# musyoku/chainer-speech-recognition

Measured on AMD Instinct MI355X. Metric: utterances/sec (T=1000, 40x3 feat, |V|~3000) CTC train step, higher is better.
Workload: dtype bf16

## Files before the change

### chainer-speech-recognition_amd/asr/_lib.py

```python
import ctypes
import os

import torch

_HERE = os.path.dirname(os.path.abspath(__file__))
_ACT = os.environ.get("ASR_ACT", "").lower()
LIB_PATH = os.environ.get("ASR_HIP_LIB") or os.path.join(os.path.dirname(_HERE),
                                                        "libasr_hip_f16.so" if _ACT in ("f16", "fp16", "float16", "half") else "libasr_hip.so")

_lib = None


def act_dtype():
    return torch.float16 if lib().asr_act_dtype() else torch.bfloat16


def debug_flag(key, default):
    for item in os.environ.get("ASR_DEBUG", "").split(","):
        k, _, v = item.strip().partition("=")
        if k == key and v:
            return int(v)
    return default

c_void_p, c_int, c_float, c_size_t = ctypes.c_void_p, ctypes.c_int, ctypes.c_float, ctypes.c_size_t
c_longlong = ctypes.c_longlong

SIGNATURES = {
    "asr_version": (c_int, []),
    "asr_act_dtype": (c_int, []),
    "asr_stream_delay": (c_int, [c_void_p, c_int]),
    "asr_occupy_cus": (c_int, [c_void_p, c_int, c_int, c_int]),
    "asr_stream_traffic": (c_int, [c_void_p, c_int, c_int, c_int, c_void_p, c_longlong]),
    "asr_ctc_workspace_bytes": (c_size_t, [c_int] * 5),
    "asr_ctc_forward": (c_int, [c_void_p] * 6 + [c_int] * 5 + [c_void_p] * 3 + [c_size_t]),
    "asr_ctc_forward_lse": (c_int, [c_void_p] * 6 + [c_int] * 5 + [c_void_p] * 3 + [c_size_t, c_void_p]),
    "asr_ctc_backward": (c_int, [c_void_p] * 3 + [c_int] * 5 + [c_void_p, c_int, c_float, c_void_p, c_void_p, c_size_t]),
    "asr_ctc_loss_grad": (c_int, [c_void_p] * 6 + [c_int] * 5 + [c_float] + [c_void_p] * 4 + [c_size_t]),
    "asr_ctc_nbest_workspace_bytes": (c_size_t, [c_int] * 5),
    "asr_ctc_nbest_forward": (c_int, [c_void_p] * 5 + [c_int] * 6 + [c_void_p, c_void_p, c_size_t]),
    "asr_ctc_nbest_backward": (c_int, [c_void_p] * 3 + [c_int] * 5 + [c_void_p] * 3 + [c_size_t]),
    "asr_specgram": (c_int, [c_void_p, c_void_p, c_int, c_void_p, c_longlong] + [c_int] * 4 + [c_float, c_void_p, c_void_p, c_int,
                               c_void_p, c_void_p, c_int, c_void_p]),
    "asr_mel_bands_bytes": (c_size_t, []),
    "asr_mel_bands": (c_int, [c_void_p, c_void_p, c_int, c_int, c_void_p, c_size_t]),
    "asr_specgram_bands": (c_int, [c_void_p, c_void_p, c_int, c_void_p, c_longlong] + [c_int] * 4 + [c_float, c_void_p, c_void_p, c_int,
                                     c_void_p, c_void_p, c_int, c_void_p, c_void_p]),
    "asr_logmel": (c_int, [c_void_p] * 3 + [c_longlong, c_int, c_int, c_void_p]),
    "asr_deltas": (c_int, [c_void_p] * 3 + [c_int] * 4 + [c_void_p] * 3),
    "asr_batchnorm_stats": (c_int, [c_void_p, c_void_p, c_longlong, c_int, c_float, c_float] + [c_void_p] * 5),
    "asr_rsqrt_eps": (c_int, [c_void_p, c_void_p, c_float, c_void_p, c_int]),
    "asr_batchnorm_fwd": (c_int, [c_void_p] * 6 + [c_longlong, c_int, c_void_p]),
    "asr_batchnorm_bwd": (c_int, [c_void_p] * 6 + [c_longlong, c_int] + [c_void_p] * 4),
    "asr_cmn_pspec": (c_int, [c_void_p] * 3 + [c_int] * 3),
    "asr_add_white_noise": (c_int, [c_void_p] * 3 + [c_longlong, c_int, c_void_p, ctypes.c_ulonglong]),
    "asr_augment_specgram": (c_int, [c_void_p] * 5 + [c_int] * 4 + [c_void_p]),
    "asr_running_stats_update": (c_int, [c_void_p] * 3 + [c_int] * 3 + [c_longlong] + [c_void_p] * 4),
    "asr_normalize_bcmt": (c_int, [c_void_p] * 4 + [c_int] * 3),
    "asr_argmax_rows": (c_int, [c_void_p, c_void_p, c_int, c_int, c_int, c_void_p]),
    "asr_ctc_collapse": (c_int, [c_void_p] * 3 + [c_int] * 4 + [c_void_p] * 2),
    "asr_edit_distance": (c_int, [c_void_p, c_void_p, c_void_p, c_int, c_void_p, c_void_p, c_int, c_int, c_void_p]),
    "asr_ctc_beam_workspace_bytes": (c_size_t, [c_int] * 5),
    "asr_ctc_beam_search": (c_int, [c_void_p] * 3 + [c_int] * 6 + [c_float, c_void_p, c_size_t] + [c_void_p] * 3),
    "asr_ngram_score": (c_int, [c_void_p] * 2 + [c_int, c_void_p, c_void_p] + [c_int] * 3 + [c_void_p] * 2 + [c_int] * 4 + [c_void_p] * 2),
    "asr_ctc_beam_lm_workspace_bytes": (c_size_t, [c_int] * 5),
    "asr_ctc_beam_search_lm": (c_int, [c_void_p] * 3 + [c_int] * 6 + [c_float, c_void_p, c_int, c_void_p, c_void_p] + [c_int] * 5
                               + [c_float, c_float, c_void_p, c_size_t] + [c_void_p] * 5),
    "asr_gram_ctc_beam_workspace_bytes": (c_size_t, [c_int] * 5),
    "asr_gram_ctc_beam_search": (c_int, [c_void_p] * 3 + [c_int] * 6 + [c_float, c_void_p, c_void_p, c_size_t] + [c_void_p] * 3),
# ... 145 lines not shown
```

### chainer-speech-recognition_amd/asr/_ops.py

```python
import os

import torch

from . import _lib
from ._lib import check, ptr, stream

BF16 = _lib.act_dtype()
F32 = torch.float32


def _is_bf16(t):
    if t.dtype == BF16:
        return 1
    if t.dtype == F32:
        return 0
    raise TypeError("expected float32 or bfloat16, got %s" % t.dtype)


def gemm_nt(a, b, bias=None, out_dtype=BF16, out=None):
    assert a.dtype == BF16 and b.dtype == BF16 and a.dim() == 2 and b.dim() == 2
    assert a.stride(1) == 1 and b.stride(1) == 1 and a.shape[1] == b.shape[1]
    M, K = a.shape
    N = b.shape[0]
    if out is None:
# ... 271 lines not shown
    y = torch.empty((rows, D), dtype=out_dtype, device=x.device)
    mean = torch.empty(rows, dtype=F32, device=x.device)
    rstd = torch.empty(rows, dtype=F32, device=x.device)
    if want_lse:
        assert x.dtype == F32 and out_dtype == F32 and _lib.lib().asr_layernorm_fwd_lse_ok(D, C)
        lse = torch.empty(rows, dtype=F32, device=x.device)
        rc = _lib.lib().asr_layernorm_fwd_lse(stream(), ptr(x), ptr(y), ptr(gamma), ptr(beta), ptr(mean), ptr(rstd), ptr(lse), rows, D)
        check(rc, "asr_layernorm_fwd_lse")
        return y, mean, rstd, lse
    rc = _lib.lib().asr_layernorm_fwd(stream(), ptr(x), _is_bf16(x), ptr(y), _is_bf16(y), ptr(gamma), ptr(beta),
                                      ptr(mean), ptr(rstd), rows, D, C)
    check(rc, "asr_layernorm_fwd")
    return y, mean, rstd


def layernorm_bwd(x, dy, gamma, mean, rstd, C, dx_dtype, dgamma=None, dbeta=None, need_dx=True):
    rows, D = x.shape
    dy = dy.contiguous()
    dx = torch.empty((rows, D), dtype=dx_dtype, device=x.device) if need_dx else None
    lib = _lib.lib()
    if x.dtype == F32 and dy.dtype == F32 and C % 4 == 0:
        nbytes = lib.asr_layernorm_bwd_rows_ws_bytes(rows, D)
        if nbytes > 0:
            ws = torch.empty(nbytes, dtype=torch.uint8, device=x.device) if dgamma is not None else None
            rc = lib.asr_layernorm_bwd_rows(stream(), ptr(x), ptr(dy), ptr(gamma), ptr(mean), ptr(rstd), ptr(dx),
                                            _is_bf16(dx) if need_dx else 0, ptr(dgamma), ptr(dbeta), rows, D, C, ptr(ws), nbytes)
            check(rc, "asr_layernorm_bwd_rows")
            return dx
    rc = lib.asr_layernorm_bwd(stream(), ptr(x), _is_bf16(x), ptr(dy), _is_bf16(dy), ptr(gamma), ptr(mean),
                               ptr(rstd), ptr(dx), _is_bf16(dx) if need_dx else 0, ptr(dgamma), ptr(dbeta),
                               rows, D, C)
    check(rc, "asr_layernorm_bwd")
    return dx


CALLS = {}


def layernorm_ctc_bwd(x, gamma, beta, mean, rstd, T, B, dx_dtype, dgamma, dbeta, need_dx, recipes, dxsum=None):
    rows, V = x.shape
    assert x.dtype == F32 and x.is_contiguous() and rows == T * B and 1 <= len(recipes) <= 2
    CALLS["layernorm_ctc_bwd"] = CALLS.get("layernorm_ctc_bwd", 0) + 1
    lib = _lib.lib()
    dx = torch.empty((rows, V), dtype=dx_dtype, device=x.device) if need_dx else None
    nbytes = lib.asr_layernorm_ctc_bwd_ws_bytes(T, B, V)
    ws = torch.empty(nbytes, dtype=torch.uint8, device=x.device) if dgamma is not None else None
    args = []
    for r in (recipes + recipes)[:2]:
        args += [ptr(r["ws"]), int(r["Lmax"]), int(r["gram"]), ptr(r["x_len"]), ptr(r["gy"]), int(r["gy_per_utt"]), float(r["scale"])]
    rc = lib.asr_layernorm_ctc_bwd(stream(), ptr(x), ptr(gamma), ptr(beta), ptr(mean), ptr(rstd), ptr(dx), _is_bf16(dx) if need_dx else 0,
                                   ptr(dgamma), ptr(dbeta), T, B, V, ptr(ws), nbytes, len(recipes), *args, ptr(dxsum))
    check(rc, "asr_layernorm_ctc_bwd")
    return dx


GRU_MODE = [int(os.environ.get("ASR_GRU_MODE", "0"))]


_SYNC = {}
_STATUS = {}


def _sync_buffer(dev, nbytes):
    key = (dev.index, torch.cuda.current_stream(dev).cuda_stream)
    buf = _SYNC.get(key)
    if buf is None or buf.numel() * 4 < nbytes:
# ... 687 lines not shown
```

### chainer-speech-recognition_amd/asr/functions.py

```python
import math
import os

import torch

from . import _ops
from ._lib import debug_flag as _lib_debug
from .link import grad_buffer, grads_queued

BF16, F32 = _ops.BF16, torch.float32


_SIDE = {"streams": {}, "origins": {}, "enabled": True, "dirty": set(), "keep": [], "keep_bytes": 0,
         "join_before_recurrence": _lib_debug("side_join", 0) != 0}
_KEEP_LIMIT = 512
_KEEP_BYTES_LIMIT = int(_lib_debug("side_keep_gb", 48)) << 30


def side_stream():
    if not _SIDE["enabled"]:
        return None
    cur = torch.cuda.current_stream()
    key = cur.cuda_stream
    st = _SIDE["streams"].get(key)
    if st is None:
        st = _SIDE["streams"][key] = torch.cuda.Stream(priority=_lib_debug("side_priority", 0))
        _SIDE["origins"][key] = cur
    return st


def side_streams():
    return list(_SIDE["streams"].values())


def join_side_stream():
    cur = torch.cuda.current_stream()
    for key, st in _SIDE["streams"].items():
        cur.wait_stream(st)
        origin = _SIDE["origins"].get(key)
        if origin is not None and origin.cuda_stream != cur.cuda_stream:
            origin.wait_stream(st)
    _SIDE["dirty"].clear()
    release_side_keeps()


def release_side_keeps(to_allocator=False):
    keep = _SIDE["keep"]
    if to_allocator:
        for t, st in keep:
            t.record_stream(st)
    del keep[:]
    _SIDE["keep_bytes"] = 0


def _empty_chip_for_recurrence():
    if not _SIDE["join_before_recurrence"] or not _SIDE["dirty"]:
        return
    cur = torch.cuda.current_stream()
    for st in _SIDE["dirty"]:
        cur.wait_stream(st)
    _SIDE["dirty"].clear()


class _OnSide(object):

# ... 53 lines not shown
    z = _ZERO.get(device)
    if z is None:
        z = _ZERO[device] = torch.zeros(1, dtype=F32, device=device)
    return z.reshape((1,) * len(shape)).expand(shape)


def _is_zero_token(t):
    z = _ZERO.get(t.device)
    return z is not None and t.data_ptr() == z.data_ptr()


def _producer_box(x2, attr="_asr_mailbox", hops=12, dtype=F32):
    if x2.dtype != dtype or not x2.is_contiguous():
        return None
    node = x2.grad_fn
    for _ in range(hops):
        if node is None:
            return None
        box = getattr(node, attr, None)
        if box is not None:
            return box if (box.ptr == x2.data_ptr() and box.numel == x2.numel()) else None
        if not type(node).__name__.startswith(_VIEW_NODES) or len(node.next_functions) != 1:
            return None
        node = node.next_functions[0][0]
    return None


def _producer_mailbox(x2):
    return _producer_box(x2, "_asr_mailbox", 8)


FUSE_CTC_INTO_LAYERNORM = [True]
LAST_FUSED_RECIPES = [0]


class _CtcBox(object):
    __slots__ = ("ptr", "numel", "shape", "recipes", "lse")

    def __init__(self, y, T, B, V, lse=None):
        self.ptr, self.numel, self.shape, self.recipes, self.lse = y.data_ptr(), y.numel(), (T, B, V), [], lse

    def post(self, recipe):
        self.recipes.append(recipe)
        return len(self.recipes) == 1

    def take(self):
        r, self.recipes = self.recipes, []
        return r


def ctc_box_of(xs):
    if not FUSE_CTC_INTO_LAYERNORM[0] or xs.dim() != 3:
        return None
    box = _producer_box(xs, "_asr_ctc_box")
    return box if (box is not None and box.shape == tuple(xs.shape)) else None


def _incoming_bf16(ctx, gy, width):
    box = getattr(ctx, "_asr_mailbox", None)
    extra = box.take() if box is not None else None
    if extra is not None and _is_zero_token(gy):
        return extra.reshape(-1, width), None
    gy = gy.contiguous()
    if gy.dtype != BF16:
        gy = _ops.cast_bf16(gy.reshape(-1, width))
    gy = gy.reshape(-1, width)
    if extra is not None:
        return _ops.add_bf16(gy, extra.reshape(-1, width)), gy
    return gy, gy


def _take_bias_done(ctx):
    done = False
# ... 690 lines not shown
    y = _SppMax.apply(p, int(pyramid_height))
    parts, o = [], 0
    for l in range(int(pyramid_height)):
        n = 4 ** l
        parts.append(y[:, o:o + n, :].permute(0, 2, 1).reshape(B, C * n))
        o += n
    return torch.cat(parts, dim=1).reshape(B, -1, 1, 1)


class _GaussianNoise(torch.autograd.Function):
    @staticmethod
    def forward(ctx, p, std, seed):
        return _ops.gaussian_noise(p, std, seed)

    @staticmethod
    def backward(ctx, gy):
        return gy, None, None


def gaussian_noise(x, std):
    if not train_mode[0]:
        return x
    p, back = _phys_any(x)
    _dropout_counter[0] += 1
    seed = (torch.initial_seed() * 1000003 + 7919 * _dropout_counter[0]) & 0xffffffff
    return back(_GaussianNoise.apply(p, float(std), seed))


class _LayerNorm(torch.autograd.Function):
    @staticmethod
    def forward(ctx, x2, gamma, beta, C, out_f32, mailbox, tb):
        per_frame = out_f32 and tb is not None and x2.dtype == F32 and C == x2.shape[1] and C % 4 == 0 and C <= 4096
        want_lse = per_frame and FUSE_CTC_INTO_LAYERNORM[0] and x2.data_ptr() % 16 == 0
        res = _ops.layernorm_fwd(x2, gamma.detach(), beta.detach(), C, F32 if out_f32 else BF16, want_lse)
        y, mean, rstd = res[:3]
        ctx.save_for_backward(x2, mean, rstd)
        ctx.params = (gamma, beta)
        ctx.meta = (C, ctx.needs_input_grad[0], mailbox)
        if per_frame:
            ctx._asr_ctc_box = _CtcBox(y, tb[0], tb[1], C, res[3] if want_lse else None)
        return y

    @staticmethod
    def backward(ctx, gy):
        x2, mean, rstd = ctx.saved_tensors
        gamma, beta = ctx.params
        C, need_dx, mailbox = ctx.meta
        handover = mailbox is not None and need_dx
        dx_dtype = BF16 if handover else x2.dtype
        box = getattr(ctx, "_asr_ctc_box", None)
        recipes = box.take() if box is not None else []
        dx = None
        if recipes:
            LAST_FUSED_RECIPES[0] = len(recipes)
            T, B, _ = box.shape
            dxsum = None
            if handover and _is_zero_token(gy) and mailbox.bias is not None and isinstance(mailbox.bias, torch.nn.Parameter) \
                    and mailbox.bias.numel() == C:
                dxsum = grad_buffer(mailbox.bias).reshape(-1)
                mailbox.bias_done = True
            dx = _ops.layernorm_ctc_bwd(x2, gamma.detach(), beta.detach(), mean, rstd, T, B, dx_dtype, grad_buffer(gamma),
                                        grad_buffer(beta), need_dx, recipes, dxsum)
        if not recipes or not _is_zero_token(gy):
            dx2 = _ops.layernorm_bwd(x2, gy.contiguous(), gamma.detach(), mean, rstd, C, dx_dtype, grad_buffer(gamma),
                                     grad_buffer(beta), need_dx)
            if dx is None:
                dx = dx2
            elif need_dx:
                dx = _ops.add_bf16(dx, dx2) if dx_dtype == BF16 else dx.add_(dx2)
        grads_queued(gamma, beta)
        if handover:
            mailbox.post(dx)
            dx = _zero_token(x2.shape, x2.device)
# ... 234 lines not shown
```

### chainer-speech-recognition_amd/asr/loss/ctc.py

```python
import collections

import torch

from .. import _lib


def _as_tbv(xs):
    if isinstance(xs, torch.Tensor):
        if xs.dim() != 3:
            raise TypeError("xs must be (T, B, V)")
        return xs
    if not isinstance(xs, (list, tuple)) or len(xs) == 0:
        raise TypeError("xs must be a list of Variables")
    whole = getattr(xs, "buffer", None)
    if whole is not None and whole.dim() == 3 and whole.shape[0] == len(xs):
        return whole
    base = getattr(xs[0], "_base", None)
    if base is not None and base.is_contiguous() and base.numel() == len(xs) * xs[0].numel() and xs[0].is_contiguous() \
            and xs[0].data_ptr() == base.data_ptr() \
            and xs[-1].data_ptr() == base.data_ptr() + (len(xs) - 1) * xs[0].numel() * base.element_size():
        return base.view((len(xs),) + tuple(xs[0].shape))
    return torch.stack(list(xs), dim=0)


class _CTCFunction(torch.autograd.Function):
    @staticmethod
    def forward(ctx, xs, label_unigram, label_bigram, input_length, label_length, blank, reduce, box):
        lib = _lib.lib()
        if xs.dtype != torch.float32:
            raise TypeError("xs must be float32")
        for t in (label_unigram, label_bigram, input_length, label_length):
            if t is not None and t.dtype != torch.int32:
                raise TypeError("labels and lengths must be int32")
        xs = xs.contiguous()
        _lib.ptr(xs)
        T, B, V = xs.shape
        Lmax = label_unigram.shape[1]
        gram = label_bigram is not None
        if gram and label_bigram.shape != label_unigram.shape:
            raise ValueError("label_unigram and label_bigram must have the same shape")
        label_unigram = label_unigram.contiguous()
        label_bigram = label_bigram.contiguous() if gram else None
        nbytes = lib.asr_ctc_workspace_bytes(T, B, V, Lmax, int(gram))
        ws = torch.empty(nbytes, dtype=torch.uint8, device=xs.device)
        loss_b = torch.empty(B, dtype=torch.float32, device=xs.device)
        loss_m = torch.empty((), dtype=torch.float32, device=xs.device)
        row_lse = box.lse if (box is not None and box.lse is not None and box.lse.numel() == T * B) else None
        rc = lib.asr_ctc_forward_lse(_lib.stream(), _lib.ptr(xs), _lib.ptr(label_unigram), _lib.ptr(label_bigram),
                                     _lib.ptr(input_length), _lib.ptr(label_length), T, B, V, Lmax, int(blank),
                                     _lib.ptr(loss_b), _lib.ptr(loss_m), _lib.ptr(ws), nbytes, _lib.ptr(row_lse))
        _lib.check(rc, "asr_ctc_forward_lse")
        ctx.save_for_backward(xs, input_length, ws)
        ctx.dims = (T, B, V, Lmax, int(gram), reduce)
        ctx.box = box if Lmax * (3 if gram else 2) + 1 <= 512 else None
        return loss_m if reduce == "mean" else loss_b

    @staticmethod
    def backward(ctx, gy):
        lib = _lib.lib()
        xs, input_length, ws = ctx.saved_tensors
        T, B, V, Lmax, gram, reduce = ctx.dims
        gy = gy.contiguous().to(torch.float32)
        scale = 1.0 / B if reduce == "mean" else 1.0
        if ctx.box is not None:
            from ..functions import _zero_token
            first = ctx.box.post(dict(ws=ws, Lmax=Lmax, gram=gram, x_len=input_length, gy=gy, gy_per_utt=0 if reduce == "mean" else 1,
                                      scale=scale))
            return (_zero_token(xs.shape, xs.device) if first else None), None, None, None, None, None, None, None
        grad = torch.empty_like(xs)
        rc = lib.asr_ctc_backward(_lib.stream(), _lib.ptr(xs), _lib.ptr(input_length), T, B, V, Lmax, gram,
                                  _lib.ptr(gy), 0 if reduce == "mean" else 1, scale, _lib.ptr(grad), _lib.ptr(ws),
                                  ws.numel())
        _lib.check(rc, "asr_ctc_backward")
        return grad, None, None, None, None, None, None, None


def _check_common(xs, blank_symbol, reduce):
    if not isinstance(blank_symbol, int):
        raise TypeError("blank_symbol must be non-negative integer.")
    if reduce not in ("mean", "no"):
        raise ValueError("only 'mean' and 'no' are valid for 'reduce', but '%s' is given" % reduce)
    x = _as_tbv(xs)
    assert blank_symbol >= 0
    assert blank_symbol < x.shape[2]
# ... 50 lines not shown
```

### chainer-speech-recognition_amd/csrc/ctc.hip

```cpp
#include "common.hpp"
#include "ctc_ws.hpp"
#include "ctc_lattice.hpp"
#include "ctc_sweep.hpp"
#include "../../include/asr_hip.h"

namespace asr {
namespace ctc {

__global__ __launch_bounds__(256) void rows_kernel(const float* __restrict__ xs, const int* __restrict__ x_len,
                                                   const int* __restrict__ path_label, int T, int B, int V, int Sp,
                                                   float* __restrict__ lse_out, float* __restrict__ lp, const float* __restrict__ lse_in) {
    __shared__ float scratch[32];
    if (lse_in) {
        const int row = blockIdx.x * 4 + (int)(threadIdx.x >> 6), lane = threadIdx.x & 63;
        if (row >= T * B) return;
        const int t = row / B, b = row - t * B;
        const int xl = x_len ? min(x_len[b], T) : T;
        if (t >= xl) return;
        const float* x = xs + (size_t)row * V;
        const float lse = lse_in[row];
        if (lane == 0) lse_out[row] = lse;
        const int* pl = path_label + (size_t)b * Sp;
        float* out = lp + ((size_t)b * T + t) * Sp;
        for (int s = lane; s < Sp; s += 64) {
            const int l = pl[s];
            out[s] = l >= 0 ? x[l] - lse : -INFINITY;
        }
        return;
    }
    const int row = blockIdx.x;
    const int t = row / B, b = row - t * B;
    const int xl = x_len ? min(x_len[b], T) : T;
    if (t >= xl) return;
    const float* x = xs + (size_t)row * V;
    float m = -INFINITY;
    const bool vec = ((V & 3) == 0) && ((((uintptr_t)x) & 15) == 0);
    if (vec) {
        const float4* x4 = reinterpret_cast<const float4*>(x);
        for (int i = threadIdx.x; i < (V >> 2); i += blockDim.x) {
            const float4 v = x4[i];
            m = fmaxf(m, fmaxf(fmaxf(v.x, v.y), fmaxf(v.z, v.w)));
        }
    } else {
        for (int i = threadIdx.x; i < V; i += blockDim.x) m = fmaxf(m, x[i]);
    }
    m = block_max(m, scratch);
    float sum = 0.f;
    if (vec) {
        const float4* x4 = reinterpret_cast<const float4*>(x);
        for (int i = threadIdx.x; i < (V >> 2); i += blockDim.x) {
            const float4 v = x4[i];
            sum += __expf(v.x - m) + __expf(v.y - m) + __expf(v.z - m) + __expf(v.w - m);
        }
    } else {
        for (int i = threadIdx.x; i < V; i += blockDim.x) sum += __expf(x[i] - m);
    }
    sum = block_sum(sum, scratch);
    const float lse = m + __logf(sum);
    if (threadIdx.x == 0) lse_out[row] = lse;
    const int* pl = path_label + (size_t)b * Sp;
    float* out = lp + ((size_t)b * T + t) * Sp;
    for (int s = threadIdx.x; s < Sp; s += blockDim.x) {
        const int l = pl[s];
        out[s] = l >= 0 ? x[l] - lse : -INFINITY;
    }
}

constexpr int kOccChunk = 8192;

__global__ __launch_bounds__(256) void grad_kernel(const float* __restrict__ xs, const int* __restrict__ x_len,
                                                   const int* __restrict__ path_label,
                                                   const int* __restrict__ path_len, const float* __restrict__ lse_in,
                                                   const double* __restrict__ alpha, const double* __restrict__ beta,
                                                   const double* __restrict__ total, const float* __restrict__ gy,
                                                   int gy_per_utt, float scale, int T, int B, int V, int Sp,
                                                   float* __restrict__ grad) {
    extern __shared__ __attribute__((aligned(16))) char smem[];
    float* occ = reinterpret_cast<float*>(smem);
    const int row = blockIdx.x;
    const int t = row / B, b = row - t * B;
    const int xl = x_len ? min(x_len[b], T) : T;
    float* g = grad + (size_t)row * V;
    const bool vec = ((V & 3) == 0) && ((((uintptr_t)g) & 15) == 0) && ((((uintptr_t)(xs + (size_t)row * V)) & 15) == 0);
    if (t >= xl) {
        if (vec) {
            float4* g4 = reinterpret_cast<float4*>(g);
            for (int i = threadIdx.x; i < (V >> 2); i += blockDim.x) g4[i] = make_float4(0.f, 0.f, 0.f, 0.f);
        } else {
            for (int i = threadIdx.x; i < V; i += blockDim.x) g[i] = 0.f;
        }
        return;
    }
    const float* x = xs + (size_t)row * V;
    const float lse = lse_in[row];
    const double tot = total[b];
    float sc = scale;
    if (gy) sc *= gy_per_utt ? gy[b] : gy[0];
// ... 26 lines not shown
                r.x = (__expf(xv.x - lse) - ov.x) * sc;
                r.y = (__expf(xv.y - lse) - ov.y) * sc;
                r.z = (__expf(xv.z - lse) - ov.z) * sc;
                r.w = (__expf(xv.w - lse) - ov.w) * sc;
                g4[i] = r;
            }
        } else {
            for (int i = threadIdx.x; i < vn; i += blockDim.x) g[v0 + i] = (__expf(x[v0 + i] - lse) - occ[i]) * sc;
        }
        __syncthreads();
    }
}

__global__ void mean_kernel(const float* __restrict__ loss, int B, float* __restrict__ out) {
    __shared__ float scratch[32];
    float s = 0.f;
    for (int i = threadIdx.x; i < B; i += blockDim.x) s += loss[i];
    s = block_sum(s, scratch);
    if (threadIdx.x == 0) out[0] = s / (float)B;
}

}
}

using namespace asr;
using namespace asr::ctc;

extern "C" size_t asr_ctc_workspace_bytes(int T, int B, int V, int Lmax, int gram) {
    (void)V;
    if (T <= 0 || B <= 0 || Lmax <= 0) return 0;
    return carve(nullptr, T, B, Lmax, gram).bytes;
}

extern "C" int asr_ctc_forward_lse(void* stream_, const float* xs, const int32_t* label_unigram,
                                   const int32_t* label_bigram, const int32_t* x_len, const int32_t* l_len, int T, int B,
                                   int V, int Lmax, int blank, float* loss_per_utt, float* loss_mean, void* workspace,
                                   size_t workspace_bytes, const float* row_lse) {
    if (!xs || !label_unigram || !loss_per_utt || !workspace) return ASR_ERR_BAD_ARG;
    if (T <= 0 || B <= 0 || V <= 0 || Lmax <= 0 || blank < 0 || blank >= V) return ASR_ERR_BAD_ARG;
    const int gram = label_bigram != nullptr;
    Workspace w = carve(workspace, T, B, Lmax, gram);
    if (workspace_bytes < w.bytes) return ASR_ERR_WORKSPACE;
    const int Sp = path_pad(Lmax, gram);
    const size_t lds = sizeof(double) * 2 * (Sp + 16) + sizeof(int) * (Sp + 8);
    if (lds > 150 * 1024) return ASR_ERR_UNSUPPORTED;
    hipStream_t stream = (hipStream_t)stream_;
    if (gram)
        hipLaunchKernelGGL(prep_kernel<true>, dim3(B), dim3(256), 0, stream, label_unigram, label_bigram, l_len, Lmax, Sp,
                           V, blank, w.path_label, w.path_mask, w.path_len);
    else
        hipLaunchKernelGGL(prep_kernel<false>, dim3(B), dim3(256), 0, stream, label_unigram, label_bigram, l_len, Lmax,
                           Sp, V, blank, w.path_label, w.path_mask, w.path_len);
    ASR_LAUNCH_CHECK();
    hipLaunchKernelGGL(rows_kernel, dim3(row_lse ? (T * B + 3) / 4 : T * B), dim3(256), 0, stream, xs, x_len, w.path_label, T, B, V, Sp, w.lse, w.lp, row_lse);
    ASR_LAUNCH_CHECK();
    const int threads = Sp < 1024 ? Sp : 1024;
    if (gram) {
        if (lds > 48 * 1024)
            (void)hipFuncSetAttribute((const void*)lattice_kernel<7>, hipFuncAttributeMaxDynamicSharedMemorySize, (int)lds);
        hipLaunchKernelGGL(lattice_kernel<7>, dim3(B, 2), dim3(threads), lds, stream, w.lp, x_len, w.path_label,
                           w.path_mask, w.path_len, T, B, Sp, w.alpha, w.beta, w.total, loss_per_utt);
    } else {
        if (lds > 48 * 1024)
            (void)hipFuncSetAttribute((const void*)lattice_kernel<3>, hipFuncAttributeMaxDynamicSharedMemorySize, (int)lds);
        hipLaunchKernelGGL(lattice_kernel<3>, dim3(B, 2), dim3(threads), lds, stream, w.lp, x_len, w.path_label,
                           w.path_mask, w.path_len, T, B, Sp, w.alpha, w.beta, w.total, loss_per_utt);
    }
    ASR_LAUNCH_CHECK();
    if (loss_mean) {
        hipLaunchKernelGGL(mean_kernel, dim3(1), dim3(256), 0, stream, loss_per_utt, B, loss_mean);
        ASR_LAUNCH_CHECK();
    }
    return ASR_OK;
}

extern "C" int asr_ctc_forward(void* stream_, const float* xs, const int32_t* label_unigram,
                               const int32_t* label_bigram, const int32_t* x_len, const int32_t* l_len, int T, int B,
                               int V, int Lmax, int blank, float* loss_per_utt, float* loss_mean, void* workspace,
                               size_t workspace_bytes) {
    return asr_ctc_forward_lse(stream_, xs, label_unigram, label_bigram, x_len, l_len, T, B, V, Lmax, blank, loss_per_utt, loss_mean,
                               workspace, workspace_bytes, nullptr);
}

extern "C" int asr_ctc_backward(void* stream_, const float* xs, const int32_t* x_len, int T, int B, int V, int Lmax,
                                int gram, const float* gy, int gy_per_utt, float scale, float* grad,
                                const void* workspace, size_t workspace_bytes) {
    if (!xs || !grad || !workspace) return ASR_ERR_BAD_ARG;
    if (T <= 0 || B <= 0 || V <= 0 || Lmax <= 0) return ASR_ERR_BAD_ARG;
    Workspace w = carve(const_cast<void*>(workspace), T, B, Lmax, gram);
    if (workspace_bytes < w.bytes) return ASR_ERR_WORKSPACE;
    const int Sp = path_pad(Lmax, gram);
    const size_t lds = sizeof(float) * (size_t)(V < kOccChunk ? (int)align_up(V, 4) : kOccChunk);
    hipStream_t stream = (hipStream_t)stream_;
    hipLaunchKernelGGL(grad_kernel, dim3(T * B), dim3(256), lds, stream, xs, x_len, w.path_label, w.path_len, w.lse,
                       w.alpha, w.beta, w.total, gy, gy_per_utt, scale, T, B, V, Sp, grad);
    ASR_LAUNCH_CHECK();
    return ASR_OK;
}

extern "C" int asr_ctc_loss_grad(void* stream, const float* xs, const int32_t* label_unigram,
                                 const int32_t* label_bigram, const int32_t* x_len, const int32_t* l_len, int T, int B,
                                 int V, int Lmax, int blank, float scale, float* loss_per_utt, float* loss_mean,
                                 float* grad, void* workspace, size_t workspace_bytes) {
    int rc = asr_ctc_forward(stream, xs, label_unigram, label_bigram, x_len, l_len, T, B, V, Lmax, blank, loss_per_utt,
                             loss_mean, workspace, workspace_bytes);
    if (rc != ASR_OK) return rc;
// ... 4 lines not shown
```

### chainer-speech-recognition_amd/csrc/layernorm.hip

```cpp
#include "common.hpp"
#include "../../include/asr_hip.h"

namespace asr {
namespace ln {

template <typename T>
__device__ __forceinline__ float ldf(const T* p, long long i) {
    if (sizeof(T) == 2) return bf16_to_f32((uint16_t)p[i]);
    return (float)p[i];
}
template <typename T>
__device__ __forceinline__ void stf(T* p, long long i, float v) {
    if (sizeof(T) == 2) p[i] = (T)f32_to_bf16(v); else p[i] = (T)v;
}

__device__ __forceinline__ float usable_rstd(float r) { return r < INFINITY ? r : 0.f; }

template <typename XT, typename YT>
__global__ __launch_bounds__(256) void fwd_kernel(const XT* __restrict__ x, YT* __restrict__ y,
                                                  const float* __restrict__ gamma, const float* __restrict__ beta,
                                                  float* __restrict__ mean_out, float* __restrict__ rstd_out, int D,
                                                  int C) {
    __shared__ float scratch[32];
    const long long row = blockIdx.x;
    const XT* xr = x + row * D;
    YT* yr = y + row * D;
    float s = 0.f;
    for (int i = threadIdx.x; i < D; i += blockDim.x) s += ldf(xr, i);
    const float mean = block_sum(s, scratch) / (float)D;
    float v = 0.f;
    for (int i = threadIdx.x; i < D; i += blockDim.x) {
        const float d = ldf(xr, i) - mean;
        v += d * d;
// ... 73 lines not shown
    float s = 0.f;
    for (int i = threadIdx.x; i < n4; i += blockDim.x) { const float4 v = xr[i]; s += (v.x + v.y) + (v.z + v.w); }
    const float mean = block_sum(s, scratch) / (float)D;
    float q = 0.f;
    for (int i = threadIdx.x; i < n4; i += blockDim.x) {
        const float4 v = xr[i];
        const float a = v.x - mean, b = v.y - mean, c = v.z - mean, d = v.w - mean;
        q += (a * a + b * b) + (c * c + d * d);
    }
    const float rstd = 1.0f / sqrtf(block_sum(q, scratch) / (float)D);
    if (threadIdx.x == 0) { mean_out[row] = mean; rstd_out[row] = rstd; }
    for (int i = threadIdx.x; i < n4; i += blockDim.x) {
        const float4 v = xr[i];
        const int c = (i * 4) % C;
        const float4 g = *reinterpret_cast<const float4*>(gamma + c), b = *reinterpret_cast<const float4*>(beta + c);
        yr[i] = make_float4((v.x - mean) * rstd * g.x + b.x, (v.y - mean) * rstd * g.y + b.y, (v.z - mean) * rstd * g.z + b.z,
                            (v.w - mean) * rstd * g.w + b.w);
    }
}
template <int NV>
__global__ __launch_bounds__(256) void fwd_rows_f32_kernel(const float* __restrict__ x, float* __restrict__ y, const float* __restrict__ gamma,
                                                           const float* __restrict__ beta, float* __restrict__ mean_out,
                                                           float* __restrict__ rstd_out, float* __restrict__ lse_out, long long rows, int D) {
    const int n4 = D >> 2, lane = threadIdx.x & 63, wid = threadIdx.x >> 6;
    float4 g[NV], b[NV];
#pragma unroll
    for (int k = 0; k < NV; ++k) {
        const int i = lane + 64 * k;
        g[k] = i < n4 ? *reinterpret_cast<const float4*>(gamma + 4 * i) : make_float4(0.f, 0.f, 0.f, 0.f);
        b[k] = i < n4 ? *reinterpret_cast<const float4*>(beta + 4 * i) : make_float4(0.f, 0.f, 0.f, 0.f);
    }
    const float inv_d = 1.0f / (float)D;
    for (long long row = (long long)blockIdx.x * 4 + wid; row < rows; row += (long long)gridDim.x * 4) {
        const float4* xr = reinterpret_cast<const float4*>(x + row * D);
        float4 v[NV];
#pragma unroll
        for (int k = 0; k < NV; ++k) {
            const int i = lane + 64 * k;
            v[k] = i < n4 ? xr[i] : make_float4(0.f, 0.f, 0.f, 0.f);
        }
        float s = 0.f;
#pragma unroll
        for (int k = 0; k < NV; ++k) s += (v[k].x + v[k].y) + (v[k].z + v[k].w);
        const float mean = wave_sum(s) * inv_d;
        float q = 0.f;
#pragma unroll
        for (int k = 0; k < NV; ++k) {
            if (lane + 64 * k < n4) {
                const float a0 = v[k].x - mean, a1 = v[k].y - mean, a2 = v[k].z - mean, a3 = v[k].w - mean;
                q += (a0 * a0 + a1 * a1) + (a2 * a2 + a3 * a3);
            }
        }
        const float rstd = 1.0f / sqrtf(wave_sum(q) * inv_d);
        if (lane == 0) { mean_out[row] = mean; rstd_out[row] = rstd; }
        float4* yr = reinterpret_cast<float4*>(y + row * D);
        float m = -INFINITY;
#pragma unroll
        for (int k = 0; k < NV; ++k) {
            const int i = lane + 64 * k;
            if (i < n4) {
                v[k] = make_float4((v[k].x - mean) * rstd * g[k].x + b[k].x, (v[k].y - mean) * rstd * g[k].y + b[k].y,
                                   (v[k].z - mean) * rstd * g[k].z + b[k].z, (v[k].w - mean) * rstd * g[k].w + b[k].w);
                yr[i] = v[k];
                m = fmaxf(m, fmaxf(fmaxf(v[k].x, v[k].y), fmaxf(v[k].z, v[k].w)));
            }
        }
        if (lse_out) {
            m = wave_max(m);
            float e = 0.f;
#pragma unroll
            for (int k = 0; k < NV; ++k)
                if (lane + 64 * k < n4) e += (__expf(v[k].x - m) + __expf(v[k].y - m)) + (__expf(v[k].z - m) + __expf(v[k].w - m));
            e = wave_sum(e);
            if (lane == 0) lse_out[row] = m + __logf(e);
        }
    }
}

__global__ __launch_bounds__(256) void bwd_f32x4_kernel(const float* __restrict__ x, const float* __restrict__ dy,
                                                        const float* __restrict__ gamma, const float* __restrict__ mean_in,
                                                        const float* __restrict__ rstd_in, float* __restrict__ dx, int D,
                                                        int C) {
    __shared__ float scratch[32];
    const long long row = blockIdx.x;
    const float4* xr = reinterpret_cast<const float4*>(x + row * D);
    const float4* gr = reinterpret_cast<const float4*>(dy + row * D);
    float4* dr = reinterpret_cast<float4*>(dx + row * D);
    const int n4 = D >> 2;
    const float mean = mean_in[row], rstd = usable_rstd(rstd_in[row]);
    float s1 = 0.f, s2 = 0.f;
    for (int i = threadIdx.x; i < n4; i += blockDim.x) {
        const float4 v = xr[i], gy = gr[i];
        const float4 gm = *reinterpret_cast<const float4*>(gamma + (i * 4) % C);
        const float g0 = gy.x * gm.x, g1 = gy.y * gm.y, g2 = gy.z * gm.z, g3 = gy.w * gm.w;
        s1 += (g0 + g1) + (g2 + g3);
        s2 += (g0 * (v.x - mean) + g1 * (v.y - mean) + g2 * (v.z - mean) + g3 * (v.w - mean)) * rstd;
    }
    const float m1 = block_sum(s1, scratch) / (float)D;
    const float m2 = block_sum(s2, scratch) / (float)D;
    for (int i = threadIdx.x; i < n4; i += blockDim.x) {
        const float4 v = xr[i], gy = gr[i];
        const float4 gm = *reinterpret_cast<const float4*>(gamma + (i * 4) % C);
        dr[i] = make_float4((gy.x * gm.x - m1 - (v.x - mean) * rstd * m2) * rstd, (gy.y * gm.y - m1 - (v.y - mean) * rstd * m2) * rstd,
                            (gy.z * gm.z - m1 - (v.z - mean) * rstd * m2) * rstd, (gy.w * gm.w - m1 - (v.w - mean) * rstd * m2) * rstd);
    }
}

// ... 488 lines not shown
```

### include/asr_hip.h

```cpp
#ifndef ASR_HIP_H
#define ASR_HIP_H
#include <stddef.h>
#include <stdint.h>
#ifdef __cplusplus
extern "C" {
#endif

int asr_version(void);
int asr_act_dtype(void);
int asr_stream_delay(void* stream, int microseconds);
int asr_occupy_cus(void* stream, int microseconds, int lds_bytes, int blocks);
int asr_stream_traffic(void* stream, int microseconds, int lds_bytes, int blocks, void* buf, long long bytes);

size_t asr_ctc_workspace_bytes(int T, int B, int V, int Lmax, int gram);
int asr_ctc_forward(void* stream, const float* xs, const int32_t* label_unigram, const int32_t* label_bigram,
                    const int32_t* x_len, const int32_t* l_len, int T, int B, int V, int Lmax, int blank,
                    float* loss_per_utt, float* loss_mean, void* workspace, size_t workspace_bytes);
int asr_ctc_forward_lse(void* stream, const float* xs, const int32_t* label_unigram, const int32_t* label_bigram,
                        const int32_t* x_len, const int32_t* l_len, int T, int B, int V, int Lmax, int blank, float* loss_per_utt,
                        float* loss_mean, void* workspace, size_t workspace_bytes, const float* row_lse);
int asr_ctc_backward(void* stream, const float* xs, const int32_t* x_len, int T, int B, int V, int Lmax, int gram,
                     const float* gy, int gy_per_utt, float scale, float* grad, const void* workspace,
                     size_t workspace_bytes);
int asr_ctc_loss_grad(void* stream, const float* xs, const int32_t* label_unigram, const int32_t* label_bigram,
                      const int32_t* x_len, const int32_t* l_len, int T, int B, int V, int Lmax, int blank, float scale,
                      float* loss_per_utt, float* loss_mean, float* grad, void* workspace, size_t workspace_bytes);
size_t asr_ctc_nbest_workspace_bytes(int T, int B, int V, int N, int Lmax);
int asr_ctc_nbest_forward(void* stream, const float* xs, const int32_t* hyp, const int32_t* hyp_len, const int32_t* x_len, int T,
                          int B, int V, int N, int Lmax, int blank, float* logp, void* workspace, size_t workspace_bytes);
int asr_ctc_nbest_backward(void* stream, const float* xs, const int32_t* x_len, int T, int B, int V, int N, int Lmax,
                           const float* gy, float* grad, const void* workspace, size_t workspace_bytes);

int asr_specgram(void* stream, const void* signals, int sig_is_f32, const int32_t* lengths, long long sig_pitch, int B,
                 int frame_len, int frame_step, int nfft, float preemph, const float* window, const int32_t* nframes,
                 int Fmax, float* pspec_out, const float* fbank, int nfilt, float* logmel_out);
size_t asr_mel_bands_bytes(void);
int asr_mel_bands(void* stream, const float* fbank, int nfilt, int nbins, void* table, size_t table_bytes);
int asr_specgram_bands(void* stream, const void* signals, int sig_is_f32, const int32_t* lengths, long long sig_pitch, int B,
                       int frame_len, int frame_step, int nfft, float preemph, const float* window, const int32_t* nframes,
                       int Fmax, float* pspec_out, const float* fbank, int nfilt, float* logmel_out, const void* bands);
int asr_logmel(void* stream, const float* pspec, const float* fbank, long long F, int nbins, int nfilt, float* out);
int asr_deltas(void* stream, const float* logmel, const int32_t* nframes, int B, int Fmax, int nfilt, int Tmax,
               const float* mean, const float* stdv, float* out);

int asr_cmn_pspec(void* stream, float* pspec, const int32_t* nframes, int B, int Fmax, int nbins);
int asr_add_white_noise(void* stream, float* signals, const int32_t* lengths, long long pitch, int B, const float* gain,
                        unsigned long long seed);
int asr_augment_specgram(void* stream, const float* pspec_in, const int32_t* nframes_out, const double* speed,
                         const double* ratio, int B, int Fmax_in, int Fmax_out, int nbins, float* pspec_out);
int asr_running_stats_update(void* stream, const float* x, const int32_t* lengths, int B, int CM, int T,
                             long long total_before, double* mean, double* nvar, float* mean32, float* std32);
int asr_normalize_bcmt(void* stream, float* x, const float* mean, const float* stdv, int B, int CM, int T);

// ... 204 lines not shown
```

Measured before the change: 2455.

## Run CTC forward on a priority loss stream, recomputing layernorm from pre-LN input

Adds a CTC forward entry point that takes the pre-layernorm activations plus gamma and beta and recomputes the normalised row, its log-sum-exp and the path log-probs inside one rows kernel. The loss head is launched on a separate high-priority stream that waits only on an event recorded before the layernorm forward, so the CTC lattice can run concurrently with the layernorm kernel rather than after it. The main stream then joins the loss stream. Shared row-wise layernorm helpers are factored into a header and reused by the existing layernorm kernel. The cost is duplicated layernorm arithmetic and reads, plus extra stream and event overhead. Workspace tensors are allocated on the side stream but consumed later on the main stream.

```diff
diff --git a/chainer-speech-recognition_amd/asr/_lib.py b/chainer-speech-recognition_amd/asr/_lib.py
--- a/chainer-speech-recognition_amd/asr/_lib.py
+++ b/chainer-speech-recognition_amd/asr/_lib.py
@@ -34,6 +34,7 @@
     "asr_ctc_workspace_bytes": (c_size_t, [c_int] * 5),
     "asr_ctc_forward": (c_int, [c_void_p] * 6 + [c_int] * 5 + [c_void_p] * 3 + [c_size_t]),
     "asr_ctc_forward_lse": (c_int, [c_void_p] * 6 + [c_int] * 5 + [c_void_p] * 3 + [c_size_t, c_void_p]),
+    "asr_ctc_forward_ln": (c_int, [c_void_p] * 8 + [c_int] * 5 + [c_void_p] * 3 + [c_size_t]),
     "asr_ctc_backward": (c_int, [c_void_p] * 3 + [c_int] * 5 + [c_void_p, c_int, c_float, c_void_p, c_void_p, c_size_t]),
     "asr_ctc_loss_grad": (c_int, [c_void_p] * 6 + [c_int] * 5 + [c_float] + [c_void_p] * 4 + [c_size_t]),
     "asr_ctc_nbest_workspace_bytes": (c_size_t, [c_int] * 5),
diff --git a/chainer-speech-recognition_amd/asr/_ops.py b/chainer-speech-recognition_amd/asr/_ops.py
--- a/chainer-speech-recognition_amd/asr/_ops.py
+++ b/chainer-speech-recognition_amd/asr/_ops.py
@@ -327,6 +327,18 @@
                                rows, D, C)
     check(rc, "asr_layernorm_bwd")
     return dx
+
+
+def ctc_forward_ln(x, gamma, beta, label_unigram, label_bigram, x_len, l_len, blank, loss_per_utt, loss_mean, ws):
+    T, B, V = x.shape
+    assert x.dtype == F32 and x.is_contiguous() and gamma.numel() == V and beta.numel() == V
+    rc = _lib.lib().asr_ctc_forward_ln(stream(), ptr(x), ptr(gamma), ptr(beta), ptr(label_unigram), ptr(label_bigram), ptr(x_len),
+                                       ptr(l_len), T, B, V, label_unigram.shape[1], int(blank), ptr(loss_per_utt), ptr(loss_mean),
+                                       ptr(ws), ws.numel())
+    if rc == -3:
+        return False
+    check(rc, "asr_ctc_forward_ln")
+    return True
 
 
 CALLS = {}
diff --git a/chainer-speech-recognition_amd/asr/functions.py b/chainer-speech-recognition_amd/asr/functions.py
--- a/chainer-speech-recognition_amd/asr/functions.py
+++ b/chainer-speech-recognition_amd/asr/functions.py
@@ -30,6 +30,19 @@
 
 def side_streams():
     return list(_SIDE["streams"].values())
+
+
+_LOSS_STREAMS = {}
+
+
+def loss_stream():
+    if not _SIDE["enabled"]:
+        return None
+    key = torch.cuda.current_stream().cuda_stream
+    st = _LOSS_STREAMS.get(key)
+    if st is None:
+        st = _LOSS_STREAMS[key] = torch.cuda.Stream(priority=-1)
+    return st
 
 
 def join_side_stream():
@@ -149,13 +162,15 @@
 
 FUSE_CTC_INTO_LAYERNORM = [True]
 LAST_FUSED_RECIPES = [0]
+SPLIT_LOSS_HEAD = [True]
+LAST_SPLIT_FORWARDS = [0]
 
 
 class _CtcBox(object):
-    __slots__ = ("ptr", "numel", "shape", "recipes", "lse")
-
-    def __init__(self, y, T, B, V, lse=None):
-        self.ptr, self.numel, self.shape, self.recipes, self.lse = y.data_ptr(), y.numel(), (T, B, V), [], lse
+    __slots__ = ("ptr", "numel", "shape", "recipes", "lse", "split")
+
+    def __init__(self, y, T, B, V, lse=None, split=None):
+        self.ptr, self.numel, self.shape, self.recipes, self.lse, self.split = y.data_ptr(), y.numel(), (T, B, V), [], lse, split
 
     def post(self, recipe):
         self.recipes.append(recipe)
@@ -912,13 +927,21 @@
     def forward(ctx, x2, gamma, beta, C, out_f32, mailbox, tb):
         per_frame = out_f32 and tb is not None and x2.dtype == F32 and C == x2.shape[1] and C % 4 == 0 and C <= 4096
         want_lse = per_frame and FUSE_CTC_INTO_LAYERNORM[0] and x2.data_ptr() % 16 == 0
+        split = None
+        if per_frame:
+            LAST_SPLIT_FORWARDS[0] = 0
+        if want_lse and SPLIT_LOSS_HEAD[0] and any(ctx.needs_input_grad) and loss_stream() is not None:
+            cur = torch.cuda.current_stream()
+            ev = torch.cuda.Event()
+            ev.record(cur)
+            split = (ev, x2, gamma.detach(), beta.detach(), cur.cuda_stream)
         res = _ops.layernorm_fwd(x2, gamma.detach(), beta.detach(), C, F32 if out_f32 else BF16, want_lse)
         y, mean, rstd = res[:3]
         ctx.save_for_backward(x2, mean, rstd)
         ctx.params = (gamma, beta)
         ctx.meta = (C, ctx.needs_input_grad[0], mailbox)
         if per_frame:
-            ctx._asr_ctc_box = _CtcBox(y, tb[0], tb[1], C, res[3] if want_lse else None)
+            ctx._asr_ctc_box = _CtcBox(y, tb[0], tb[1], C, res[3] if want_lse else None, split)
         return y
 
     @staticmethod
diff --git a/chainer-speech-recognition_amd/asr/loss/ctc.py b/chainer-speech-recognition_amd/asr/loss/ctc.py
--- a/chainer-speech-recognition_amd/asr/loss/ctc.py
+++ b/chainer-speech-recognition_amd/asr/loss/ctc.py
@@ -39,17 +39,39 @@
         gram = label_bigram is not None
         if gram and label_bigram.shape != label_unigram.shape:
             raise ValueError("label_unigram and label_bigram must have the same shape")
+        as_given = all(t is None or t.is_contiguous() for t in (label_unigram, label_bigram, input_length, label_length))
         label_unigram = label_unigram.contiguous()
         label_bigram = label_bigram.contiguous() if gram else None
         nbytes = lib.asr_ctc_workspace_bytes(T, B, V, Lmax, int(gram))
-        ws = torch.empty(nbytes, dtype=torch.uint8, device=xs.device)
-        loss_b = torch.empty(B, dtype=torch.float32, device=xs.device)
-        loss_m = torch.empty((), dtype=torch.float32, device=xs.device)
         row_lse = box.lse if (box is not None and box.lse is not None and box.lse.numel() == T * B) else None
-        rc = lib.asr_ctc_forward_lse(_lib.stream(), _lib.ptr(xs), _lib.ptr(label_unigram), _lib.ptr(label_bigram),
-                                     _lib.ptr(input_length), _lib.ptr(label_length), T, B, V, Lmax, int(blank),
-                                     _lib.ptr(loss_b), _lib.ptr(loss_m), _lib.ptr(ws), nbytes, _lib.ptr(row_lse))
-        _lib.check(rc, "asr_ctc_forward_lse")
+        done = False
+        split = box.split if (box is not None and row_lse is not None) else None
+        cur = torch.cuda.current_stream()
+        if split is not None and split[4] == cur.cuda_stream and as_given:
+            from .. import _ops, functions
+            side = functions.loss_stream()
+            if side is not None:
+                ev, x2, gamma, beta, _ = split
+                try:
+                    with torch.cuda.stream(side):
+                        side.wait_event(ev)
+                        ws = torch.empty(nbytes, dtype=torch.uint8, device=xs.device)
+                        loss_b = torch.empty(B, dtype=torch.float32, device=xs.device)
+                        loss_m = torch.empty((), dtype=torch.float32, device=xs.device)
+                        done = _ops.ctc_forward_ln(x2.view(T, B, V), gamma, beta, label_unigram, label_bigram, input_length, label_length,
+                                                   blank, loss_b, loss_m, ws)
+                finally:
+                    cur.wait_stream(side)
+                if done:
+                    functions.LAST_SPLIT_FORWARDS[0] += 1
+        if not done:
+            ws = torch.empty(nbytes, dtype=torch.uint8, device=xs.device)
+            loss_b = torch.empty(B, dtype=torch.float32, device=xs.device)
+            loss_m = torch.empty((), dtype=torch.float32, device=xs.device)
+            rc = lib.asr_ctc_forward_lse(_lib.stream(), _lib.ptr(xs), _lib.ptr(label_unigram), _lib.ptr(label_bigram),
+                                         _lib.ptr(input_length), _lib.ptr(label_length), T, B, V, Lmax, int(blank),
+                                         _lib.ptr(loss_b), _lib.ptr(loss_m), _lib.ptr(ws), nbytes, _lib.ptr(row_lse))
+            _lib.check(rc, "asr_ctc_forward_lse")
         ctx.save_for_backward(xs, input_length, ws)
         ctx.dims = (T, B, V, Lmax, int(gram), reduce)
         ctx.box = box if Lmax * (3 if gram else 2) + 1 <= 512 else None
diff --git a/chainer-speech-recognition_amd/csrc/ctc.hip b/chainer-speech-recognition_amd/csrc/ctc.hip
--- a/chainer-speech-recognition_amd/csrc/ctc.hip
+++ b/chainer-speech-recognition_amd/csrc/ctc.hip
@@ -2,6 +2,7 @@
 #include "ctc_ws.hpp"
 #include "ctc_lattice.hpp"
 #include "ctc_sweep.hpp"
+#include "ln_row.hpp"
 #include "../../include/asr_hip.h"
 
 namespace asr {
@@ -63,6 +64,42 @@
     for (int s = threadIdx.x; s < Sp; s += blockDim.x) {
         const int l = pl[s];
         out[s] = l >= 0 ? x[l] - lse : -INFINITY;
+    }
+}
+
+template <int NV>
+__global__ __launch_bounds__(256) void rows_ln_kernel(const float* __restrict__ x, const float* __restrict__ gamma,
+                                                      const float* __restrict__ beta, const int* __restrict__ x_len,
+                                                      const int* __restrict__ path_label, int T, int B, int V, int Sp,
+                                                      float* __restrict__ lse_out, float* __restrict__ lp) {
+    const int n4 = V >> 2, lane = threadIdx.x & 63, wid = threadIdx.x >> 6;
+    float4 g[NV], b[NV];
+#pragma unroll
+    for (int k = 0; k < NV; ++k) {
+        const int i = lane + 64 * k;
+        g[k] = i < n4 ? *reinterpret_cast<const float4*>(gamma + 4 * i) : make_float4(0.f, 0.f, 0.f, 0.f);
+        b[k] = i < n4 ? *reinterpret_cast<const float4*>(beta + 4 * i) : make_float4(0.f, 0.f, 0.f, 0.f);
+    }
+    const float inv_d = 1.0f / (float)V;
+    const long long rows = (long long)T * B;
+    for (long long row = (long long)blockIdx.x * 4 + wid; row < rows; row += (long long)gridDim.x * 4) {
+        const int t = (int)(row / B), bb = (int)(row - (long long)t * B);
+        const int xl = x_len ? min(x_len[bb], T) : T;
+        if (t >= xl) continue;
+        const float* xr = x + row * V;
+        float4 v[NV];
+        ln::row_load<NV>(xr, lane, n4, v);
+        float mean, rstd;
+        ln::row_stats<NV>(v, lane, n4, inv_d, mean, rstd);
+        const float m = ln::row_normalise<NV, false>(v, g, b, mean, rstd, lane, n4, nullptr);
+        const float lse = ln::row_lse<NV>(v, m, lane, n4);
+        if (lane == 0) lse_out[row] = lse;
+        const int* pl = path_label + (size_t)bb * Sp;
+        float* out = lp + ((size_t)bb * T + t) * Sp;
+        for (int s = lane; s < Sp; s += 64) {
+            const int l = pl[s];
+            out[s] = l >= 0 ? __fsub_rn(ln::row_affine(xr[l], mean, rstd, gamma[l], beta[l]), lse) : -INFINITY;
+        }
     }
 }
 
@@ -155,10 +192,10 @@
     return carve(nullptr, T, B, Lmax, gram).bytes;
 }
 
-extern "C" int asr_ctc_forward_lse(void* stream_, const float* xs, const int32_t* label_unigram,
-                                   const int32_t* label_bigram, const int32_t* x_len, const int32_t* l_len, int T, int B,
-                                   int V, int Lmax, int blank, float* loss_per_utt, float* loss_mean, void* workspace,
-                                   size_t workspace_bytes, const float* row_lse) {
+static int forward_launch(void* stream_, const float* xs, const float* gamma, const float* beta, const int32_t* label_unigram,
+                          const int32_t* label_bigram, const int32_t* x_len, const int32_t* l_len, int T, int B,
+                          int V, int Lmax, int blank, float* loss_per_utt, float* loss_mean, void* workspace,
+                          size_t workspace_bytes, const float* row_lse) {
     if (!xs || !label_unigram || !loss_per_utt || !workspace) return ASR_ERR_BAD_ARG;
     if (T <= 0 || B <= 0 || V <= 0 || Lmax <= 0 || blank < 0 || blank >= V) return ASR_ERR_BAD_ARG;
     const int gram = label_bigram != nullptr;
@@ -175,7 +212,16 @@
         hipLaunchKernelGGL(prep_kernel<false>, dim3(B), dim3(256), 0, stream, label_unigram, label_bigram, l_len, Lmax,
                            Sp, V, blank, w.path_label, w.path_mask, w.path_len);
     ASR_LAUNCH_CHECK();
-    hipLaunchKernelGGL(rows_kernel, dim3(row_lse ? (T * B + 3) / 4 : T * B), dim3(256), 0, stream, xs, x_len, w.path_label, T, B, V, Sp, w.lse, w.lp, row_lse);
+    if (gamma) {
+        long long blocks = ((long long)T * B + 3) / 4;
+        if (blocks > 256 * 3) blocks = 256 * 3;
+        const int nv = cdiv(V >> 2, 64);
+#define ASR_RLN(NV) hipLaunchKernelGGL(rows_ln_kernel<NV>, dim3((unsigned)blocks), dim3(256), 0, stream, xs, gamma, beta, x_len, w.path_label, T, B, V, Sp, w.lse, w.lp)
+        if (nv <= 4) ASR_RLN(4); else if (nv <= 8) ASR_RLN(8); else if (nv <= 12) ASR_RLN(12); else ASR_RLN(16);
+#undef ASR_RLN
+    } else {
+        hipLaunchKernelGGL(rows_kernel, dim3(row_lse ? (T * B + 3) / 4 : T * B), dim3(256), 0, stream, xs, x_len, w.path_label, T, B, V, Sp, w.lse, w.lp, row_lse);
+    }
     ASR_LAUNCH_CHECK();
     const int threads = Sp < 1024 ? Sp : 1024;
     if (gram) {
@@ -195,6 +241,25 @@
         ASR_LAUNCH_CHECK();
     }
     return ASR_OK;
+}
+
+extern "C" int asr_ctc_forward_lse(void* stream_, const float* xs, const int32_t* label_unigram,
+                                   const int32_t* label_bigram, const int32_t* x_len, const int32_t* l_len, int T, int B,
+                                   int V, int Lmax, int blank, float* loss_per_utt, float* loss_mean, void* workspace,
+                                   size_t workspace_bytes, const float* row_lse) {
+    return forward_launch(stream_, xs, nullptr, nullptr, label_unigram, label_bigram, x_len, l_len, T, B, V, Lmax, blank, loss_per_utt,
+                          loss_mean, workspace, workspace_bytes, row_lse);
+}
+
+extern "C" int asr_ctc_forward_ln(void* stream_, const float* x, const float* gamma, const float* beta, const int32_t* label_unigram,
+                                  const int32_t* label_bigram, const int32_t* x_len, const int32_t* l_len, int T, int B,
+                                  int V, int Lmax, int blank, float* loss_per_utt, float* loss_mean, void* workspace,
+                                  size_t workspace_bytes) {
+    if (!gamma || !beta) return ASR_ERR_BAD_ARG;
+    if (V > 0 && ((V & 3) || V > 4096)) return ASR_ERR_UNSUPPORTED;
+    if ((((uintptr_t)x) | ((uintptr_t)gamma) | ((uintptr_t)beta)) & 15) return ASR_ERR_UNSUPPORTED;
+    return forward_launch(stream_, x, gamma, beta, label_unigram, label_bigram, x_len, l_len, T, B, V, Lmax, blank, loss_per_utt,
+                          loss_mean, workspace, workspace_bytes, nullptr);
 }
 
 extern "C" int asr_ctc_forward(void* stream_, const float* xs, const int32_t* label_unigram,
diff --git a/chainer-speech-recognition_amd/csrc/layernorm.hip b/chainer-speech-recognition_amd/csrc/layernorm.hip
--- a/chainer-speech-recognition_amd/csrc/layernorm.hip
+++ b/chainer-speech-recognition_amd/csrc/layernorm.hip
@@ -1,4 +1,5 @@
 #include "common.hpp"
+#include "ln_row.hpp"
 #include "../../include/asr_hip.h"
 
 namespace asr {
@@ -138,47 +139,15 @@
     }
     const float inv_d = 1.0f / (float)D;
     for (long long row = (long long)blockIdx.x * 4 + wid; row < rows; row += (long long)gridDim.x * 4) {
-        const float4* xr = reinterpret_cast<const float4*>(x + row * D);
         float4 v[NV];
-#pragma unroll
-        for (int k = 0; k < NV; ++k) {
-            const int i = lane + 64 * k;
-            v[k] = i < n4 ? xr[i] : make_float4(0.f, 0.f, 0.f, 0.f);
-        }
-        float s = 0.f;
-#pragma unroll
-        for (int k = 0; k < NV; ++k) s += (v[k].x + v[k].y) + (v[k].z + v[k].w);
-        const float mean = wave_sum(s) * inv_d;
-        float q = 0.f;
-#pragma unroll
-        for (int k = 0; k < NV; ++k) {
-            if (lane + 64 * k < n4) {
-                const float a0 = v[k].x - mean, a1 = v[k].y - mean, a2 = v[k].z - mean, a3 = v[k].w - mean;
-                q += (a0 * a0 + a1 * a1) + (a2 * a2 + a3 * a3);
-            }
-        }
-        const float rstd = 1.0f / sqrtf(wave_sum(q) * inv_d);
+        row_load<NV>(x + row * D, lane, n4, v);
+        float mean, rstd;
+        row_stats<NV>(v, lane, n4, inv_d, mean, rstd);
         if (lane == 0) { mean_out[row] = mean; rstd_out[row] = rstd; }
-        float4* yr = reinterpret_cast<float4*>(y + row * D);
-        float m = -INFINITY;
-#pragma unroll
-        for (int k = 0; k < NV; ++k) {
-            const int i = lane + 64 * k;
-            if (i < n4) {
-                v[k] = make_float4((v[k].x - mean) * rstd * g[k].x + b[k].x, (v[k].y - mean) * rstd * g[k].y + b[k].y,
-                                   (v[k].z - mean) * rstd * g[k].z + b[k].z, (v[k].w - mean) * rstd * g[k].w + b[k].w);
-                yr[i] = v[k];
-                m = fmaxf(m, fmaxf(fmaxf(v[k].x, v[k].y), fmaxf(v[k].z, v[k].w)));
-            }
-        }
+        const float m = row_normalise<NV, true>(v, g, b, mean, rstd, lane, n4, y + row * D);
         if (lse_out) {
-            m = wave_max(m);
-            float e = 0.f;
-#pragma unroll
-            for (int k = 0; k < NV; ++k)
-                if (lane + 64 * k < n4) e += (__expf(v[k].x - m) + __expf(v[k].y - m)) + (__expf(v[k].z - m) + __expf(v[k].w - m));
-            e = wave_sum(e);
-            if (lane == 0) lse_out[row] = m + __logf(e);
+            const float lse = row_lse<NV>(v, m, lane, n4);
+            if (lane == 0) lse_out[row] = lse;
         }
     }
 }
diff --git a/chainer-speech-recognition_amd/csrc/ln_row.hpp b/chainer-speech-recognition_amd/csrc/ln_row.hpp
--- /dev/null
+++ b/chainer-speech-recognition_amd/csrc/ln_row.hpp
@@ -0,0 +1,69 @@
+#pragma once
+#include "common.hpp"
+
+namespace asr {
+namespace ln {
+
+__device__ __forceinline__ float row_affine(float x, float mean, float rstd, float g, float b) {
+    return __fmaf_rn(__fmul_rn(__fsub_rn(x, mean), rstd), g, b);
+}
+
+template <int NV>
+__device__ __forceinline__ void row_load(const float* __restrict__ x_row, int lane, int n4, float4 (&v)[NV]) {
+    const float4* xr = reinterpret_cast<const float4*>(x_row);
+#pragma unroll
+    for (int k = 0; k < NV; ++k) {
+        const int i = lane + 64 * k;
+        v[k] = i < n4 ? xr[i] : make_float4(0.f, 0.f, 0.f, 0.f);
+    }
+}
+
+template <int NV>
+__device__ __forceinline__ void row_stats(const float4 (&v)[NV], int lane, int n4, float inv_d, float& mean, float& rstd) {
+    float s = 0.f;
+#pragma unroll
+    for (int k = 0; k < NV; ++k) s += (v[k].x + v[k].y) + (v[k].z + v[k].w);
+    mean = __fmul_rn(wave_sum(s), inv_d);
+    float q = 0.f;
+#pragma unroll
+    for (int k = 0; k < NV; ++k) {
+        if (lane + 64 * k < n4) {
+            const float a0 = __fsub_rn(v[k].x, mean), a1 = __fsub_rn(v[k].y, mean), a2 = __fsub_rn(v[k].z, mean), a3 = __fsub_rn(v[k].w, mean);
+            q += __fmaf_rn(a0, a0, __fmul_rn(a1, a1)) + __fmaf_rn(a2, a2, __fmul_rn(a3, a3));
+        }
+    }
+    rstd = 1.0f / sqrtf(__fmul_rn(wave_sum(q), inv_d));
+}
+
+template <int NV, bool STORE>
+__device__ __forceinline__ float row_normalise(float4 (&v)[NV], const float4 (&g)[NV], const float4 (&b)[NV], float mean, float rstd,
+                                               int lane, int n4, float* __restrict__ y_row) {
+    float4* yr = reinterpret_cast<float4*>(y_row);
+    float m = -INFINITY;
+#pragma unroll
+    for (int k = 0; k < NV; ++k) {
+        const int i = lane + 64 * k;
+        if (i < n4) {
+            v[k] = make_float4(row_affine(v[k].x, mean, rstd, g[k].x, b[k].x), row_affine(v[k].y, mean, rstd, g[k].y, b[k].y),
+                               row_affine(v[k].z, mean, rstd, g[k].z, b[k].z), row_affine(v[k].w, mean, rstd, g[k].w, b[k].w));
+            if (STORE) yr[i] = v[k];
+            m = fmaxf(m, fmaxf(fmaxf(v[k].x, v[k].y), fmaxf(v[k].z, v[k].w)));
+        }
+    }
+    return m;
+}
+
+template <int NV>
+__device__ __forceinline__ float row_lse(const float4 (&v)[NV], float m, int lane, int n4) {
+    m = wave_max(m);
+    float e = 0.f;
+#pragma unroll
+    for (int k = 0; k < NV; ++k)
+        if (lane + 64 * k < n4)
+            e += (__expf(__fsub_rn(v[k].x, m)) + __expf(__fsub_rn(v[k].y, m))) + (__expf(__fsub_rn(v[k].z, m)) + __expf(__fsub_rn(v[k].w, m)));
+    e = wave_sum(e);
+    return m + __logf(e);
+}
+
+}
+}
diff --git a/include/asr_hip.h b/include/asr_hip.h
--- a/include/asr_hip.h
+++ b/include/asr_hip.h
@@ -19,6 +19,9 @@
 int asr_ctc_forward_lse(void* stream, const float* xs, const int32_t* label_unigram, const int32_t* label_bigram,
                         const int32_t* x_len, const int32_t* l_len, int T, int B, int V, int Lmax, int blank, float* loss_per_utt,
                         float* loss_mean, void* workspace, size_t workspace_bytes, const float* row_lse);
+int asr_ctc_forward_ln(void* stream, const float* x, const float* gamma, const float* beta, const int32_t* label_unigram,
+                       const int32_t* label_bigram, const int32_t* x_len, const int32_t* l_len, int T, int B, int V, int Lmax,
+                       int blank, float* loss_per_utt, float* loss_mean, void* workspace, size_t workspace_bytes);
 int asr_ctc_backward(void* stream, const float* xs, const int32_t* x_len, int T, int B, int V, int Lmax, int gram,
                      const float* gy, int gy_per_utt, float scale, float* grad, const void* workspace,
                      size_t workspace_bytes);
```

After: 2441. Within noise of the previous version (-0.6%).
